# Nithin-Holla/meme_challenge

Measured on AMD Instinct MI355X. Metric: train samples/sec UNITER-base (36 regions, 128 tok), higher is better.
Workload: dtype f32

## Files before the change

### include/uniter_hip.h

```cpp
#ifndef UNITER_HIP_H
#define UNITER_HIP_H

#include <stddef.h>
#include <stdint.h>

#ifdef __cplusplus
extern "C" {
#endif

#define UNITER_ABI_VERSION 1

#define UNITER_E_ARG   (-1)
#define UNITER_E_SHAPE (-2)
#define UNITER_E_WS    (-3)
#define UNITER_E_STATE (-4)

int         uniter_abi_version(void);
const char* uniter_last_error(void);
const char* uniter_build_info(void);

enum {
  UNITER_EPI_NONE      = 0,
  UNITER_EPI_BIAS      = 1,
  UNITER_EPI_BIAS_GELU = 2,
// ... 67 lines not shown
                  void* stream);
int uniter_join3(const void* x3, int rows, int cols, size_t row_stride, size_t piece_stride, float* x, int ld,
                 void* stream);
int uniter_gemm_x3_cfg(int cfg, int nsplit, int a_kmajor, int b_kmajor, int M, int N, int K, const void* A, int lda,
                       int psa, const void* B, int ldb, int psb, float* C, int ldc, long c_split_stride, void* C_x3,
                       int ldcx, int pscx, int epilogue, const float* bias, const float* aux_in, float* aux_out,
                       int ld_aux, void* stream);
int uniter_gemm_x3_plan(int M, int N, int K, int avail_cus, int nsplit_fixed, int* cfg, int* nsplit);
int uniter_gemm_x3_plan_fwd32(int M, int N, int K, int avail_cus, int nsplit_fixed, int* cfg, int* nsplit);
int uniter_wgrad_x3_group(int cfg, int n, const int* M, const int* N, int K, const void* const* A,
                          const void* const* B, float* const* dW, int overwrite, int max_wgs, void* stream);
typedef struct uniter_x3_riders {
  double* ssq;
  float* colsum_out;
  int grid, njobs, nred;
  const float* part[4];
  int nparts[4], stride[4], n[4], seg[4];
  float* out[4][3];
  int first_item[5];
} uniter_x3_riders_t;
int uniter_gemm_x3_colpart(int cfg, int a_kmajor, int b_kmajor, int M, int N, int K, const void* A, int lda, int psa,
                           const void* B, int ldb, int psb, float* C, int ldc, void* C_x3, int ldcx, int pscx,
                           const float* aux_in, int ld_aux, float* colsum_part, void* stream);
int uniter_wgrad_x3_group_riders(int cfg, int n, const int* M, const int* N, int K, const void* const* A,
                                 const void* const* B, float* const* dW, int overwrite, int max_wgs,
                                 uniter_x3_riders_t* riders, void* stream);
int uniter_wgrad_x3_group_slots(int cfg, int n, const int* M, const int* N, int max_wgs);
size_t uniter_gemm_x3_balanced_ws_bytes(void);
int uniter_gemm_x3_cfg_ws(int cfg, int nsplit, int a_kmajor, int b_kmajor, int M, int N, int K, const void* A, int lda,
                          int psa, const void* B, int ldb, int psb, float* C, int ldc, long c_split_stride, void* C_x3,
                          int ldcx, int pscx, int epilogue, const float* bias, const float* aux_in, float* aux_out,
                          int ld_aux, void* ws, size_t ws_bytes, void* stream);
int uniter_wgrad_x3_group_ws(int cfg, int n, const int* M, const int* N, int K, const void* const* A,
                             const void* const* B, float* const* dW, int overwrite, int max_wgs,
                             uniter_x3_riders_t* riders, void* ws, size_t ws_bytes, void* stream);
int uniter_wgrad_x3_group_slots_ws(int cfg, int n, const int* M, const int* N, int K, int max_wgs, size_t ws_bytes);
int uniter_wgrad_bf16_group_riders(int cfg, int n, const int* M, const int* N, int K, const void* const* A,
                                   const void* const* B, float* const* dW, int overwrite, int max_wgs,
                                   uniter_x3_riders_t* riders, void* stream);
int uniter_wgrad_bf16_group_slots(int n, const int* M, const int* N, int max_wgs);
int uniter_wgrad_bf16_group_slots_cfg(int cfg, int n, const int* M, const int* N, int max_wgs);
int uniter_gemm_bf16p_plan(int M, int N, int K, int avail_cus, int nsplit_fixed, int b_kmajor, int* cfg, int* nsplit);
int uniter_gemm_bf16p_colpart(int b_kmajor, int M, int N, int K, const void* A, int lda, const void* B, int ldb, float* C, int ldc,
                              void* C_bf16, int ldcb, const void* aux_in, int aux_in_bf16, int ld_aux, float* colsum_part,
                              void* stream);
int uniter_colsum_x3_add(const void* x3, int rows, int cols, int ldx, float* out, void* stream);
// ... 426 lines not shown
```

### meme_challenge_amd/_lib.py

```python
import ctypes as C
import os

import torch

_HERE = os.path.dirname(os.path.abspath(__file__))
LIB_PATH = os.path.join(_HERE, 'libuniter_hip.so')
if os.environ.get('UNITER_LIB_VARIANT'):
    LIB_PATH = os.path.join(_HERE, 'libuniter_hip_%s.so' % os.environ['UNITER_LIB_VARIANT'])

c_f32p = C.c_void_p
c_i64p = C.c_void_p
c_u8p = C.c_void_p


class UniterConfigC(C.Structure):
    _fields_ = [('hidden_size', C.c_int32), ('num_hidden_layers', C.c_int32),
                ('num_attention_heads', C.c_int32), ('intermediate_size', C.c_int32),
                ('vocab_size', C.c_int32), ('max_position_embeddings', C.c_int32),
                ('type_vocab_size', C.c_int32), ('img_dim', C.c_int32),
                ('hidden_dropout_prob', C.c_float),
                ('attention_probs_dropout_prob', C.c_float)]


class X3RidersC(C.Structure):
# ... 50 lines not shown
    'uniter_slab_reduce_add': (_I, [_P, _I, _SZ, _P, _SZ, _P]),
    'uniter_colsum_bf16_add': (_I, [_P, _I, _I, _I, _P, _P]),
    'uniter_colsum_bf16_add_det': (_I, [_P, _I, _I, _I, _P, _P, _SZ, _P]),
    'uniter_colsum_det_ws_bytes': (_SZ, [_I, _I]),
    'uniter_wgrad_bf16_group': (_I, [_I, _I, _P, _P, _I, _P, _P, _P, _P]),
    'uniter_wgrad_f32_group': (_I, [_I, _P, _P, _I, _P, _P, _P, _I, _P]),
    'uniter_ln_bwd_b16': (_I, [_P, _P, _P, _P, _P, _P, _P, _P, _P, _P, _P, _I, _I, _F, _U64, _U32, _U32, _P, _SZ, _P]),
    'uniter_ln_bwd_rows': (_I, [_P, _P, _P, _P, _P, _P, _P, _P, _I, _I, _I, _F, _U64, _U32, _U32, _P, _SZ, _P]),
    'uniter_ln_bwd_finalize': (_I, [_P, _SZ, _I, _I, _P, _P, _P, _P]),
    'uniter_ln_bwd': (_I, [_P, _P, _P, _P, _P, _P, _P, _P, _P, _P, _I, _I, _F, _U64, _U32, _U32, _P, _SZ, _P]),
    'uniter_ln_bwd_ws_bytes': (_SZ, [_I, _I]),
    'uniter_attn_fwd': (_I, [_P, _P, _P, _P, _I, _I, _I, _F, _U64, _U32, _U32, _P]),
    'uniter_gemm_bf16res_cfg': (_I, [_I, _I, _I, _I, _I, _I, _P, _I, _P, _I, _P, _I, _P, _I, _I, _P, _P, _P, _I, _I, _P]),
    'uniter_gemm_bf16v2_cfg': (_I, [_I, _I, _I, _I, _I, _I, _I, _P, _I, _P, _I, _P, _I, C.c_long, _P, _I, _I, _P, _P, _I, _P, _I, _I, _I, _P]),
    'uniter_split3': (_I, [_P, _I, _I, _I, _P, _SZ, _SZ, _P]),
    'uniter_join3': (_I, [_P, _I, _I, _SZ, _SZ, _P, _I, _P]),
    'uniter_gemm_x3_cfg': (_I, [_I, _I, _I, _I, _I, _I, _I, _P, _I, _I, _P, _I, _I, _P, _I, C.c_long, _P, _I, _I, _I, _P, _P, _P, _I, _P]),
    'uniter_ln_fwd_slabs_x3': (_I, [_P, _I, _SZ, _P, _P, _P, _P, _P, _P, _P, _P, _I, _I, _F, _U64, _U32, _U32, _P]),
    'uniter_ln_bwd_rows_slabs_x3': (_I, [_P, _I, _SZ, _P, _P, _P, _P, _P, _P, _P, _I, _I, _I, _F, _U64, _U32, _U32, _P, _SZ, _P]),
    'uniter_wgrad_x3_group': (_I, [_I, _I, _P, _P, _I, _P, _P, _P, _I, _I, _P]),
    'uniter_gemm_x3_plan': (_I, [_I, _I, _I, _I, _I, _P, _P]),
    'uniter_gemm_x3_plan_fwd32': (_I, [_I, _I, _I, _I, _I, _P, _P]),
    'uniter_gemm_x3_colpart': (_I, [_I, _I, _I, _I, _I, _I, _P, _I, _I, _P, _I, _I, _P, _I, _P, _I, _I, _P, _I, _P, _P]),
    'uniter_wgrad_x3_group_riders': (_I, [_I, _I, _P, _P, _I, _P, _P, _P, _I, _I, _P, _P]),
    'uniter_wgrad_x3_group_slots': (_I, [_I, _I, _P, _P, _I]),
    'uniter_gemm_x3_balanced_ws_bytes': (_SZ, []),
    'uniter_gemm_x3_cfg_ws': (_I, [_I, _I, _I, _I, _I, _I, _I, _P, _I, _I, _P, _I, _I, _P, _I, C.c_long, _P, _I, _I, _I, _P, _P, _P, _I, _P, _SZ, _P]),
    'uniter_wgrad_x3_group_ws': (_I, [_I, _I, _P, _P, _I, _P, _P, _P, _I, _I, _P, _P, _SZ, _P]),
    'uniter_wgrad_x3_group_slots_ws': (_I, [_I, _I, _P, _P, _I, _I, _SZ]),
    'uniter_wgrad_bf16_group_riders': (_I, [_I, _I, _P, _P, _I, _P, _P, _P, _I, _I, _P, _P]),
    'uniter_wgrad_bf16_group_slots': (_I, [_I, _P, _P, _I]),
    'uniter_wgrad_bf16_group_slots_cfg': (_I, [_I, _I, _P, _P, _I]),
    'uniter_gemm_bf16p_plan': (_I, [_I, _I, _I, _I, _I, _I, _P, _P]),
    'uniter_gemm_bf16p_colpart': (_I, [_I, _I, _I, _I, _P, _I, _P, _I, _P, _I, _P, _I, _P, _I, _I, _P, _P]),
    'uniter_hidden_keep_bits_bytes': (_SZ, [_SZ]),
    'uniter_hidden_keep_bits_gen': (_I, [_P, _SZ, _I, _U32, _U32, _U32, _SZ, _F, _U64, _U32, _P]),
    'uniter_ln_set_next_keep_bits': (_I, [_P]),
    'uniter_model_set_norm_partials': (_I, [_P, _P, _SZ]),
    'uniter_model_set_aux_stream': (_I, [_P, _P]),
    'uniter_model_set_cu_reserve': (_I, [_P, _I]),
    'uniter_model_set_deterministic': (_I, [_P, _I]),
    'uniter_model_deterministic_coverage': (_I, [_P]),
    'uniter_attn_bwd_set_next_det': (_I, [_I]),
    'uniter_model_norm_partials_per_layer': (_I, [_P]),
    'uniter_colsum_x3_add': (_I, [_P, _I, _I, _I, _P, _P]),
    'uniter_colsum_x3_add_det': (_I, [_P, _I, _I, _I, _P, _P, _SZ, _P]),
# ... 223 lines not shown
```

### meme_challenge_amd/csrc/gemm_internal.h

```cpp
#pragma once
#include "common.h"

struct GemmOperand {
  const void* p = nullptr;
  int ld = 0, piece_stride = 0, kmajor = 0;
};
struct GemmCall {
  int M = 0, N = 0, K = 0;
  GemmOperand A, B;
  float* C = nullptr;
  int ldc = 0, nsplit = 1;
  long c_split_stride = 0;
  void* Ccopy = nullptr;
  int ld_copy = 0, ps_copy = 0;
  int epi = UNITER_EPI_NONE;
  const float* bias = nullptr;
  const void* aux_in = nullptr;
  void* aux_out = nullptr;
  int aux_in_bf16 = 0, aux_out_bf16 = 0, ld_aux = 0;
  int beta = 0, no_sk = 0;
  float* colpart = nullptr;
  void* sk_ws = nullptr;
  size_t sk_ws_bytes = 0;
  void* stream = nullptr;
// ... 12 lines not shown
  return 0;
}
static inline bool gemm_side_buffers_aligned(const GemmCall& c) {
  return c.ldc % 4 == 0 && c.ld_copy % 8 == 0 && c.ld_aux % 4 == 0 && ((uintptr_t)c.C & 15) == 0 && ((uintptr_t)c.Ccopy & 15) == 0 &&
         ((uintptr_t)c.aux_in & 15) == 0 && ((uintptr_t)c.aux_out & 15) == 0 && ((uintptr_t)c.bias & 15) == 0;
}
static inline bool gemm_f32_side_in_range(const GemmCall& c, int pad) {
  return ((size_t)c.M + pad) * (c.ldc > 0 ? c.ldc : 1) * 4 < (1ull << 31) && ((size_t)c.M + pad) * (c.ld_aux > 0 ? c.ld_aux : 1) * 4 < (1ull << 31);
}

int gemm_f32_run(int cfg, int tag, const GemmCall& c, const LaunchOpts& lo);
int gemm_bf16_run(int cfg, const GemmCall& c, const LaunchOpts& lo);
int gemm_bf16res_run(int cfg, const GemmCall& c, const LaunchOpts& lo);
int gemm_bf16v2_run(int cfg, const GemmCall& c, const LaunchOpts& lo);
int gemm_b1p_run(int cfg, const GemmCall& c, const LaunchOpts& lo);
int gemm_x3_run(int cfg, const GemmCall& c, const LaunchOpts& lo);
size_t gemm_x3_sk_ws_bytes();
int gemm_x3_wgrad_default_cfg();
int gemm_x3_pick_split(int M, int N, int K);
int gemm_x3_pick_split_on(int M, int N, int K, int avail, int cu_reserve);
int gemm_bf16v2_pick_split(int M, int N, int K);
int gemm_b1p_pick_split(int M, int N, int K, int avail, int cu_reserve);
int gemm_bf16v2_wgrad_pieces(int M, int N, int K);

struct WgradGroupCall {
  int n = 0, K = 0;
  const int* Kp = nullptr;
  const int *Mo = nullptr, *No = nullptr;
  const void *const *A = nullptr, *const *B = nullptr;
  float* const* dW = nullptr;
  int overwrite = 0, max_wgs = 0;
  uniter_x3_riders_t* riders = nullptr;
  void *sk_ws = nullptr, *stream = nullptr;
  size_t sk_ws_bytes = 0;
};
int gemm_f32_wgrad_group(const WgradGroupCall& c, const LaunchOpts& lo);
int gemm_bf16v2_wgrad_group(int cfg, const WgradGroupCall& c, const LaunchOpts& lo);
int gemm_b1p_wgrad_group(const WgradGroupCall& c, const LaunchOpts& lo);
int gemm_x3_wgrad_group(int cfg, const WgradGroupCall& c, const LaunchOpts& lo);
int gemm_x3_wgrad_group_slots(int cfg, int n, const int* Mo, const int* No, int max_wgs, int K, size_t sk_ws_bytes, int cu_reserve);
int gemm_x3_wgrad_group_balanced_wgs(int cfg, int n, const int* Mo, const int* No, int cu_reserve);
int gemm_b1p_wgrad_group_slots(int n, const int* Mo, const int* No, int max_wgs, int cu_reserve);
int gemm_bf16v2_wgrad_group_slots(int n, const int* Mo, const int* No, int max_wgs, int cu_reserve);
int gemm_bf16v2_wgrad_group_balanced_wgs(int n, const int* Mo, const int* No, int cu_reserve);

static inline int wgrad_group_check(const char* who, const WgradGroupCall& c) {
// ... 68 lines not shown
```

### meme_challenge_amd/csrc/model.cpp

```cpp
#include <stdlib.h>
#include <string.h>
#include <algorithm>
#include <string>
#include <vector>
#include "common.h"
#include "gemm_internal.h"
#include "philox.h"
#include "switches.h"

namespace {

enum { P_WORD = 0, P_POS, P_TYPE, P_ELN_G, P_ELN_B, P_IMG_W, P_IMG_B, P_ILN_G, P_ILN_B, P_PLN_G, P_PLN_B,
       P_POSL_W, P_POSL_B, P_MASK_EMB, P_FLN_G, P_FLN_B, P_LAYER0 };
enum { L_QW = 0, L_QB, L_KW, L_KB, L_VW, L_VB, L_OW, L_OB, L_LN1_G, L_LN1_B, L_W1, L_B1, L_W2, L_B2, L_LN2_G,
       L_LN2_B, L_COUNT };

const char* kEmbNames[P_LAYER0] = {
    "embeddings.word_embeddings.weight", "embeddings.position_embeddings.weight",
    "embeddings.token_type_embeddings.weight", "embeddings.LayerNorm.weight", "embeddings.LayerNorm.bias",
    "img_embeddings.img_linear.weight", "img_embeddings.img_linear.bias",
    "img_embeddings.img_layer_norm.weight", "img_embeddings.img_layer_norm.bias",
    "img_embeddings.pos_layer_norm.weight", "img_embeddings.pos_layer_norm.bias",
    "img_embeddings.pos_linear.weight", "img_embeddings.pos_linear.bias",
    "img_embeddings.mask_embedding.weight", "img_embeddings.LayerNorm.weight", "img_embeddings.LayerNorm.bias"};
// ... 37 lines not shown
  AttnKernel attn_fwd, attn_bwd;
  float *feat_eff, *imgfc, *img_stats, *cat, *emb;
  std::vector<LayerBufs> layers;
  float *dcat, *d_imgfc, *d_posfc, *d_feat, *dsum, *dpk;
  unsigned short* embb;
  Precision prec = PREC_F32;
  bool copies() const { return prec >= PREC_BF16; }
  int ns_kh;
  int ns_ki_b, ns_kh_b, ns_k3h_b;
  int ns_ki, ns_k3h;
  bool packed;
  bool det;
  int wg_group;
  float* wg_slabs;
  unsigned char* hid_keepb;
  size_t hid_stride;
  bool hid_on;
  void *ln_ws, *col_ws, *emb_ws, *attn_ws;
  void *emb_ws2, *emb_ws3;
  size_t ln_ws_bytes, col_ws_bytes, emb_ws_bytes, attn_ws_bytes;
  void *sk_main, *sk_side;
  size_t sk_bytes;
  bool head_rows = false;
  int hr_ns_h = 1, hr_ns_i = 1;
  LayerBufs hr;
  float *hr_x = nullptr, *hr_dy = nullptr;
  size_t total;
};

}

struct uniter_model {
  uniter_config_t cfg;
  int n_params;
  std::vector<float*> p, g;
  std::vector<std::string> names;
  std::vector<hipEvent_t> ev_main, ev_side, ev_mid;
  Precision precision = PREC_F32;
  bool mirror_paired = false;
  const unsigned short* mirror = nullptr;
  const float* mirror_base = nullptr;
  size_t mirror_numel = 0;
  const unsigned short* WB(int l, int k) const { return mirror + (LP(l, k) - mirror_base); }
  std::vector<hipEvent_t> ready;
  int prof_kind = 0;
  std::vector<hipEvent_t> prof_ev;
// ... 114 lines not shown
      b.dz2 = cv.f(M * H); b.g2 = cv.f(M * H); b.du = cv.f(M * I); b.dy1 = cv.f(s_ki_b * M * H); b.dz1 = cv.f(M * H);
      b.g1 = cv.f(M * H); b.dctx = cv.f(s_kh_b * M * H); b.dqkv = cv.f(M * 3 * H); b.delta = cv.f((size_t)B * nh * L);
      b.dx = cv.f(s_k3h * M * H);
      b.du_csum = cv.f((size_t)((M + 31) / 32) * I);
      b.qb_part = cv.f((size_t)B * 3 * H);
      b.keepb = (unsigned short*)cv.raw(uniter_attn_keep_bits_bytes(B, L, nh));
      b.ln_ws1 = cv.raw(uniter_ln_bwd_ws_bytes(pl.M, H));
      b.ln_ws2 = cv.raw(uniter_ln_bwd_ws_bytes(pl.M, H));
      if (pl.copies()) { b.g2b = cv.h(pc * M * H); b.dub = cv.h(pc * M * I); b.g1b = cv.h(pc * M * H); b.dqkvb = cv.h(pc * M * 3 * H); }
    }
  } else {
    LayerBufs base = LayerBufs();
    alloc_fwd(base);
    float* yB = cv.f(M * H);
    for (int l = 0; l < nl; ++l) {
      pl.layers[l] = base;
      if (l & 1) pl.layers[l].y2 = yB;
    }
  }
  pl.sk_bytes = gemm_x3_sk_ws_bytes();
  pl.sk_main = (x3 && (sw.x3_balanced & 2)) ? cv.raw(pl.sk_bytes) : nullptr;
  pl.sk_side = (x3 && save && (sw.x3_balanced & 1)) ? cv.raw(pl.sk_bytes) : nullptr;
  pl.head_rows = false;
  pl.hr = LayerBufs(); pl.hr_x = pl.hr_dy = nullptr;
  if (x3 && !pl.packed) {
    const size_t Bc = (size_t)B;
    LayerBufs& h = pl.hr;
    auto pieces_for = [](int K) { const int n = K / 32 / 2; return n < 1 ? 1 : (n > 8 ? 8 : n); };
    pl.hr_ns_h = pieces_for(H); pl.hr_ns_i = pieces_for(I);
    const size_t s_h = (size_t)pl.hr_ns_h, s_i = (size_t)pl.hr_ns_i;
    h.ctx = cv.f(Bc * H); h.ctxb = cv.h(pc * Bc * H); pl.hr_x = cv.f(Bc * H); h.t1 = cv.f(s_h * Bc * H);
    h.z1 = save ? cv.f(Bc * H) : nullptr; h.mean1 = cv.f(Bc); h.rstd1 = cv.f(Bc); h.y1 = cv.f(Bc * H); h.y1b = cv.h(pc * Bc * H);
    h.u = save ? cv.f(Bc * I) : nullptr; h.hact = cv.f(Bc * I); h.hactb = cv.h(pc * Bc * I); h.t2 = cv.f(s_i * Bc * H);
    h.z2 = save ? cv.f(Bc * H) : nullptr; h.mean2 = cv.f(Bc); h.rstd2 = cv.f(Bc); h.y2 = cv.f(Bc * H);
    if (save) {
      pl.hr_dy = cv.f(Bc * H); h.dz2 = cv.f(Bc * H); h.g2b = cv.h(pc * Bc * H); h.dub = cv.h(pc * Bc * I); h.dy1 = cv.f(s_i * Bc * H);
      h.dz1 = cv.f(Bc * H); h.g1b = cv.h(pc * Bc * H); h.dctx = cv.f(Bc * H);
      h.du_csum = cv.f((size_t)((Bc + 31) / 32) * I);
      h.ln_ws1 = cv.raw(uniter_ln_bwd_ws_bytes(B, H));
      h.ln_ws2 = cv.raw(uniter_ln_bwd_ws_bytes(B, H));
    }
  }
  if (save) {
    pl.hid_stride = align_up(uniter_hidden_keep_bits_bytes(M * H), 256);
    pl.hid_keepb = (unsigned char*)cv.raw(pl.hid_stride * 2 * nl);
    pl.dcat = cv.f((size_t)B * pl.S * H);
    pl.d_imgfc = cv.f(BR * H);
    pl.d_posfc = cv.f(BR * H);
    pl.d_feat = has_masks ? cv.f(BR * c.img_dim) : nullptr;
    pl.dsum = cv.f(M * H);
    pl.dpk = cv.f(M * H);
    pl.ln_ws_bytes = uniter_ln_bwd_ws_bytes(pl.M, H);
    pl.ln_ws = cv.raw(pl.ln_ws_bytes);
    const int maxN = 3 * H > I ? 3 * H : I;
    pl.col_ws_bytes = uniter_colsum_ws_bytes(pl.M, maxN);
    pl.col_ws = cv.raw(pl.col_ws_bytes);
    const int rows = B * (T > R ? T : R);
    pl.emb_ws_bytes = uniter_embed_bwd_ws_bytes(rows, H);
    pl.det = m->deterministic;
    if (pl.det) {
      const size_t d = uniter_embed_bwd_det_ws_bytes(has_txt ? B * T : 0, (int)BR, H);
      if (d > pl.emb_ws_bytes) pl.emb_ws_bytes = d;
    }
// ... 78 lines not shown
    const int cfg = (kind == UNITER_K_GEMM_FFN_UP_FWD && sw.x3_cfg_ffn_up_fwd) ? sw.x3_cfg_ffn_up_fwd : sw.x3_cfg;
    const LaunchOpts lo = {ps.stamp, sw.main_prio_x3, m->launch_reserve};
    g.A = {a.b, 3 * K, K, 0}; g.B.piece_stride = (int)m->mirror_numel; g.ld_copy = 3 * N; g.ps_copy = N; g.ld_aux = N;
    g.sk_ws = pl.sk_main; g.sk_ws_bytes = pl.sk_main ? pl.sk_bytes : 0;
    return gemm_x3_run(cfg | (m->mirror_paired ? 64 : 0), g, lo);
  }
  const LaunchOpts lo = {ps.stamp, sw.main_prio_bf16, m->launch_reserve};
  g.A = {a.b, K, 0, 0}; g.ld_copy = c.b ? N : 0; g.ld_aux = ld_aux;
  g.aux_in_bf16 = epi == UNITER_EPI_MUL || epi == UNITER_EPI_DGELU; g.aux_out_bf16 = epi == UNITER_EPI_BIAS_GELU || epi == UNITER_EPI_BIAS_GELU_D;
  int cfg = 0;
  const int mask = sw.b16_persist;
  const bool epi_ok = epi == UNITER_EPI_NONE || epi == UNITER_EPI_BIAS || epi == UNITER_EPI_ADD || epi == UNITER_EPI_BIAS_GELU_D || epi == UNITER_EPI_MUL;
  if (epi_ok && K % 64 == 0) {
    if ((mask & 1) && kind == UNITER_K_GEMM_QKV_FWD && !bkm && N % 192 == 0) cfg = 8;
    else if ((mask & 2) && pieces > 1 && N <= 1024) cfg = 6;
    else if ((mask & 8) && pieces == 1 && N >= 2048) cfg = 7;
  }
  if (colpart) {
    UCHECK_ARG(epi_ok && K % 64 == 0 && pieces == 1, "linear: column partials ride on the persistent kernels");
    return gemm_b1p_run(7, g, lo);
  }
  return gemm_bf16v2_run(cfg, g, lo);
}
AttnKernel attn_kernel(const Plan& pl, float p_drop, bool save, bool keep_pre, bool bwd) {
  const Switches& sw = uniter_switches();
  const bool fused = pl.L <= uniter_attn_varlen_max_len();
  const bool pieces = pl.L <= uniter_attn_x3_max_len() && (p_drop == 0.f || keep_pre || bwd);
  if (pl.prec == PREC_BF16 && fused) return (sw.attn_b16x && pieces) ? ATTN_B16X : ATTN_BF16_PRE;
  if (pl.prec == PREC_X3 && sw.attn_x3 && pieces && (fused || !bwd)) return ATTN_X3;
  if (pl.prec == PREC_X3 && fused) return ATTN_F32_PRE_X3;
  if (pl.packed || (save && fused)) return ATTN_F32_PRE;
  return ATTN_F32;
}
int x3_backward_cus(const uniter_model* m) {
  const int a = (gemm_chip_cus() - m->cu_reserve) / 8 * 8;
  return a >= 8 ? a : 8;
}
struct WgradGroup {
  bool riders = false;
  bool colpart = false;
  int cfg = 0, max_wgs = 0, slots = 0;
};
WgradGroup wgrad_group(const uniter_model* m, const Plan& pl, int l, int cu_reserve, bool own_k = false) {
  const Switches& sw = uniter_switches();
  const int H = m->cfg.hidden_size, I = m->cfg.intermediate_size;
  const int Mo[4] = {I, H, 3 * H, H}, No[4] = {H, I, H, H};
// ... 141 lines not shown
  if (pl.det) {
    const LayerBufs& lb = rows != pl.M ? pl.hr : pl.layers[l];
    return (x3 ? uniter_colsum_x3_add_det : uniter_colsum_bf16_add_det)(t.A[0], rows, t.Mo[0], t.Mo[0], m->LG(l, L_B1), lb.du_csum,
                                                                       du_csum_bytes(rows, t.Mo[0]), sd);
  }
  return (x3 ? uniter_colsum_x3_add : uniter_colsum_bf16_add)(t.A[0], rows, t.Mo[0], t.Mo[0], m->LG(l, L_B1), sd);
}

int head_rows_gather(void* dst, const void* src, int B, int L, size_t row_bytes, hipStream_t st) {
  UCHECK_HIP(hipMemcpy2DAsync(dst, row_bytes, src, (size_t)L * row_bytes, row_bytes, (size_t)B, hipMemcpyDeviceToDevice, st));
  return 0;
}
int head_rows_scatter(void* dst, const void* src, int B, int L, size_t row_bytes, hipStream_t st) {
  UCHECK_HIP(hipMemcpy2DAsync(dst, (size_t)L * row_bytes, src, row_bytes, row_bytes, (size_t)B, hipMemcpyDeviceToDevice, st));
  return 0;
}
int head_rows_forward(uniter_model* m, hipStream_t st, int l, Act x, float* hidden_out, float ph) {
  Plan& pl = m->plan;
  const int H = m->cfg.hidden_size, I = m->cfg.intermediate_size, B = pl.B, L = pl.L;
  const LayerBufs& lb = pl.layers[l];
  LayerBufs& h = pl.hr;
  const bool save = pl.mode != 0;
  const size_t rowb = (size_t)H * sizeof(float);
  UCHECK_RC(head_rows_gather(h.ctx, lb.ctx, B, L, rowb, st));
  UCHECK_RC(head_rows_gather(pl.hr_x, x.f, B, L, rowb, st));
  const Act ctx = {h.ctx, h.ctxb}, y1 = {h.y1, h.y1b}, hact = {h.hact, h.hactb};
  UCHECK_RC(operand_copy(pl, ctx, B, H, st));
  UCHECK_RC(linear(m, UNITER_K_GEMM_ATTN_OUT_FWD, st, 0, B, H, H, l, L_OW, ctx, Act{h.t1, nullptr}, pl.hr_ns_h, UNITER_EPI_BIAS, m->LP(l, L_OB), nullptr,
                   nullptr));
  UCHECK_RC(ln_fwd(m, st, l, 0, h.t1, pl.hr_ns_h, pl.hr_x, h.z1, y1, h.mean1, h.rstd1, ph, B, L));
  float* gelu_aux = save ? h.u : h.hact;
  UCHECK_RC(linear(m, UNITER_K_GEMM_FFN_UP_FWD, st, 0, B, I, H, l, L_W1, y1, hact, 1, UNITER_EPI_BIAS_GELU_D, m->LP(l, L_B1), nullptr, gelu_aux));
  UCHECK_RC(linear(m, UNITER_K_GEMM_FFN_DOWN_FWD, st, 0, B, H, I, l, L_W2, hact, Act{h.t2, nullptr}, pl.hr_ns_i, UNITER_EPI_BIAS, m->LP(l, L_B2), nullptr,
                   nullptr));
  UCHECK_RC(ln_fwd(m, st, l, 1, h.t2, pl.hr_ns_i, h.y1, h.z2, Act{h.y2, nullptr}, h.mean2, h.rstd2, ph, B, L));
  UCHECK_HIP(hipMemsetAsync(hidden_out, 0, (size_t)B * L * rowb, st));
  return head_rows_scatter(hidden_out, h.y2, B, L, rowb, st);
}

int validate_batch(const uniter_model* m, const uniter_batch_t* b) {
  UCHECK_ARG(b, "batch is NULL");
  UCHECK_ARG(b->B > 0 && b->L > 0, "batch: B and L must be positive");
  UCHECK_ARG(b->input_ids || b->img_feat, "batch: need input_ids and/or img_feat");
  UCHECK_ARG(b->attention_mask, "batch: attention_mask is NULL");
  if (b->input_ids) UCHECK_ARG(b->position_ids && b->T > 0, "batch: text needs position_ids and T > 0");
  if (b->img_feat) UCHECK_ARG(b->img_pos_feat && b->R > 0, "batch: image needs img_pos_feat and R > 0");
  const int S = (b->input_ids ? b->T : 0) + (b->img_feat ? b->R : 0);
  if (!(b->input_ids && b->img_feat && b->gather_index))
    UCHECK_SHAPE(b->L == S || (b->input_ids && b->img_feat && b->L <= S),
                 "batch: without gather_index L (%d) must equal T+R (%d)", b->L, S);
  UCHECK_SHAPE(b->T <= m->cfg.max_position_embeddings || !b->input_ids, "batch: T exceeds max_position_embeddings");
  return 0;
}

}

extern "C" int uniter_num_params(const uniter_config_t* cfg) {
// ... 347 lines not shown
  const float* dh = nullptr;
  if (l == nl - 1 || m->all_layers) {
    dh = m->d_hidden + (m->all_layers ? (size_t)l * ((size_t)B * L * H) : 0);
    if (pl.packed) {
      UCHECK_RC(uniter_row_gather(dh, m->batch.pack_dst, pl.dpk, M, H, B * L, st));
      dh = pl.dpk;
    }
  }
  const bool hr = pl.head_rows && l == nl - 1;
  LayerBufs& pb = hr ? pl.hr : lb;
  const int Mp = hr ? B : M, row_step = hr ? L : 1;
  if (hr) {
    UCHECK_RC(head_rows_gather(pl.hr_dy, dh, B, L, (size_t)H * sizeof(float), st));
    dy = pl.hr_dy;
  } else if (l == nl - 1) {
    dy = dh;
  } else if (m->all_layers) {
    UCHECK_RC(launch_add_f32(pl.dsum, pl.layers[l + 1].dx, dh, MH, st));
    dy = pl.dsum;
  } else {
    dy = pl.layers[l + 1].dx;
  }
  const bool copies = pl.copies();
  const Act g2 = {ph > 0.f ? (copies ? nullptr : pb.g2) : pb.dz2, pb.g2b};
  const Act g1 = {ph > 0.f ? (copies ? nullptr : pb.g1) : pb.dz1, pb.g1b};
  const int ns_dy = (l == nl - 1 || m->all_layers) ? 1 : pl.ns_k3h;
  const int ns_dx = (l == 0 || m->all_layers) ? 1 : pl.ns_k3h;
  UCHECK_RC(ln_bwd(m, st, l, 1, dy, ns_dy, pb.z2, pb.mean2, pb.rstd2, pb.dz2, g2, pb.ln_ws2, ph, hr ? Mp : 0, row_step));
  const bool fuse_db1 = H % 64 == 0;
  const Switches& sw = uniter_switches();
  const bool attn_b16 = attn_is_b16(pl.attn_bwd);
  const bool fused_qb = pl.attn_bwd != ATTN_F32;
  const int ns_dctx = hr ? 1 : (pl.attn_bwd == ATTN_X3 && sw.dctx_split) ? pl.ns_kh_b : 1;
  const int ns_dy1 = hr ? pl.hr_ns_i : pl.ns_ki_b;
  const int epi_du = pl.gelu_d ? UNITER_EPI_MUL : UNITER_EPI_DGELU;
  const WgradGroup wg = copies ? wgrad_group(m, pl, l, m->launch_reserve, hr && Mp != M) : WgradGroup();
  const Act du = {pb.du, pb.dub}, dqkv = {lb.dqkv, lb.dqkvb};
  UCHECK_RC(linear(m, UNITER_K_GEMM_DGRAD, st, 1, Mp, I, H, l, L_W2, g2, du, 1, epi_du, nullptr, pb.u, nullptr,
                   (copies ? wg.colpart : fuse_db1) ? pb.du_csum : nullptr));
  UCHECK_RC(linear(m, UNITER_K_GEMM_DGRAD, st, 1, Mp, H, I, l, L_W1, du, Act{pb.dy1, nullptr}, ns_dy1, UNITER_EPI_ADD, nullptr, pb.dz2,
                   nullptr));
  UCHECK_RC(ln_bwd(m, st, l, 0, pb.dy1, ns_dy1, pb.z1, pb.mean1, pb.rstd1, pb.dz1, g1, pb.ln_ws1, ph, hr ? Mp : 0, row_step));
  const WgradProducts wp = {{I, H, 3 * H, H}, {H, I, H, H}, {pb.dub, pb.g2b, lb.dqkvb, pb.g1b}, {pb.y1b, pb.hactb, x.b, pb.ctxb},
                            {m->LG(l, L_W1), m->LG(l, L_W2), m->LG(l, L_QW), m->LG(l, L_OW)}, {Mp, Mp, M, Mp}};
  const int wp_all[4] = {0, 1, 2, 3}, wp_early[3] = {0, 1, 3}, wp_late[1] = {2};
  const bool wg_early = pl.prec == PREC_BF16 && pl.wg_group >= 2 && sd != st;
  if (wg_early) {
    UCHECK_HIP(hipEventRecord(m->ev_mid[l], st));
    UCHECK_HIP(hipStreamWaitEvent(sd, m->ev_mid[l], 0));
    UCHECK_RC(wgrad_launch(m, l, sd, wp, wp_early, 3, 1, 0, nullptr, true));
  }
  UCHECK_RC(linear(m, UNITER_K_GEMM_DGRAD, st, 1, Mp, H, H, l, L_OW, g1, Act{pb.dctx, nullptr}, ns_dctx, UNITER_EPI_NONE, nullptr, nullptr,
                   nullptr));
  if (hr) {
    const size_t rowb = (size_t)H * sizeof(float);
    UCHECK_HIP(hipMemsetAsync(lb.dctx, 0, MH * sizeof(float), st));
    UCHECK_RC(head_rows_scatter(lb.dctx, pb.dctx, B, L, rowb, st));
    UCHECK_HIP(hipMemsetAsync(lb.dz1, 0, MH * sizeof(float), st));
    UCHECK_RC(head_rows_scatter(lb.dz1, pb.dz1, B, L, rowb, st));
  }
  if (m->ag.out) {
    const uniter_model::AttnGrads& ag = m->ag;
    UCHECK_RC(uniter_attn_grad(lb.qkv, attn_b16 ? 1 : 0, pl.packed ? nullptr : m->batch.attention_mask, pl.packed ? m->batch.cu_seqlens : nullptr,
                               lb.dctx, ns_dctx, MH, ag.out + (size_t)l * ag.stride,
                               ag.head_sums ? ag.head_sums + (size_t)l * B * nh : nullptr, ag.ws, ag.ws_bytes, B, L, nh, ag.reduce, st));
  }
  {
    ProfScope ps(m, UNITER_K_ATTN_BWD, st);
    const AttnKernel k = pl.attn_bwd;
    const bool flags_only = attn_reads_flags_only(k);
    AttnCall c;
    c.B = B; c.L = L; c.nh = nh; c.qkv = lb.qkv; c.qkv_is_bf16 = attn_b16;
    c.mask = pl.packed ? nullptr : m->batch.attention_mask; c.cu_seqlens = pl.packed ? m->batch.cu_seqlens : nullptr;
    c.ctx = lb.ctx; c.lse = lb.lse; c.p_drop = pa; c.stream = st;
    c.keep_bits = fused_qb ? lb.keepb : nullptr;
    c.seed = flags_only ? 0 : m->seed; c.offset = flags_only ? 0 : m->offset; c.site = flags_only ? 0 : SITE_ATTN_PROBS(l);
// ... 462 lines not shown
```

Before: 1701.

## Add skinny fp32 MFMA GEMM for head-rows last-layer linears

Adds a dedicated skinny GEMM kernel (M<=64) that uses fp32 MFMA with per-wave k-splitting and an LDS reduction, with fused bias/GELU/add/mul epilogues. The last layer's head-rows path uses it for forward and dgrad linears on the few gathered rows. It reads ctx straight through a strided lda, which removes a gather and an operand split copy. The intent is to cut launch and tiling overhead of general GEMMs on tiny-M shapes. In exchange it allocates extra fp32 gradient buffers and adds a second code path whose accuracy and x3 copy handling must match the old one.

```diff
diff --git a/include/uniter_hip.h b/include/uniter_hip.h
--- a/include/uniter_hip.h
+++ b/include/uniter_hip.h
@@ -113,6 +113,9 @@
 int uniter_gemm_x3_colpart(int cfg, int a_kmajor, int b_kmajor, int M, int N, int K, const void* A, int lda, int psa,
                            const void* B, int ldb, int psb, float* C, int ldc, void* C_x3, int ldcx, int pscx,
                            const float* aux_in, int ld_aux, float* colsum_part, void* stream);
+int uniter_gemm_skinny(int b_kmajor, int M, int N, int K, const float* A, int lda, const float* W, int ldw, float* C, int ldc,
+                       long c_split_stride, int nsplit, void* C_x3, int ldcx, int pscx, int epilogue, const float* bias,
+                       const float* aux_in, float* aux_out, int ld_aux, float* colsum_part, void* stream);
 int uniter_wgrad_x3_group_riders(int cfg, int n, const int* M, const int* N, int K, const void* const* A,
                                  const void* const* B, float* const* dW, int overwrite, int max_wgs,
                                  uniter_x3_riders_t* riders, void* stream);
diff --git a/meme_challenge_amd/_lib.py b/meme_challenge_amd/_lib.py
--- a/meme_challenge_amd/_lib.py
+++ b/meme_challenge_amd/_lib.py
@@ -96,6 +96,7 @@
     'uniter_gemm_x3_plan': (_I, [_I, _I, _I, _I, _I, _P, _P]),
     'uniter_gemm_x3_plan_fwd32': (_I, [_I, _I, _I, _I, _I, _P, _P]),
     'uniter_gemm_x3_colpart': (_I, [_I, _I, _I, _I, _I, _I, _P, _I, _I, _P, _I, _I, _P, _I, _P, _I, _I, _P, _I, _P, _P]),
+    'uniter_gemm_skinny': (_I, [_I, _I, _I, _I, _P, _I, _P, _I, _P, _I, C.c_long, _I, _P, _I, _I, _I, _P, _P, _P, _I, _P, _P]),
     'uniter_wgrad_x3_group_riders': (_I, [_I, _I, _P, _P, _I, _P, _P, _P, _I, _I, _P, _P]),
     'uniter_wgrad_x3_group_slots': (_I, [_I, _I, _P, _P, _I]),
     'uniter_gemm_x3_balanced_ws_bytes': (_SZ, []),
diff --git a/meme_challenge_amd/csrc/gemm_internal.h b/meme_challenge_amd/csrc/gemm_internal.h
--- a/meme_challenge_amd/csrc/gemm_internal.h
+++ b/meme_challenge_amd/csrc/gemm_internal.h
@@ -58,6 +58,9 @@
 int gemm_bf16v2_pick_split(int M, int N, int K);
 int gemm_b1p_pick_split(int M, int N, int K, int avail, int cu_reserve);
 int gemm_bf16v2_wgrad_pieces(int M, int N, int K);
+int gemm_skinny_run(const GemmCall& c, const LaunchOpts& lo);
+bool gemm_skinny_takes(int M, int N, int K);
+int gemm_skinny_pick_split(int K);
 
 struct WgradGroupCall {
   int n = 0, K = 0;
diff --git a/meme_challenge_amd/csrc/head_rows.hip b/meme_challenge_amd/csrc/head_rows.hip
--- /dev/null
+++ b/meme_challenge_amd/csrc/head_rows.hip
@@ -0,0 +1,208 @@
+#include "bf16_tile.h"
+#include "gemm_internal.h"
+
+namespace {
+
+constexpr int SK_WAVES = 8;
+
+struct SkArgs {
+  int M, N, K;
+  const float* A; int lda;
+  const float* W; int ldw;
+  float* C; int ldc; long c_split_stride; int nsplit;
+  unsigned short* Cx; int ldcx, pscx;
+  const float* bias; const float* aux_in; float* aux_out; int ld_aux;
+  float* colpart;
+  int strips;
+  unsigned long long* stamp;
+};
+
+enum { SK_NONE = 0, SK_BIAS, SK_BIAS_GELU_D, SK_ADD, SK_MUL };
+
+__device__ __forceinline__ f32x4 ld4(const float* p, bool ok) {
+  return ok ? *reinterpret_cast<const f32x4*>(p) : f32x4{0.f, 0.f, 0.f, 0.f};
+}
+
+template <int BKM, int RB>
+__global__ __launch_bounds__(64 * SK_WAVES) void skinny_kernel(const SkArgs g, const int epi) {
+  constexpr int SN = BKM ? 32 : 16, KU = BKM ? 16 : 32, NB = BKM ? 2 : 1, ROWS = 16 * RB;
+  __shared__ __attribute__((aligned(16))) float part[SK_WAVES * ROWS * SN];
+  const int lane = threadIdx.x & 63, wave = threadIdx.x >> 6, r = lane & 15, q = lane >> 4;
+  const int piece = blockIdx.x / g.strips, n0 = (blockIdx.x - piece * g.strips) * SN;
+  stamp_begin(g.stamp);
+  const int units = (g.K + KU - 1) / KU;
+  const int u0 = (int)((long)units * piece / g.nsplit), u1 = (int)((long)units * (piece + 1) / g.nsplit);
+  f32x4 acc[RB][NB];
+#pragma unroll
+  for (int b = 0; b < RB; ++b)
+#pragma unroll
+    for (int j = 0; j < NB; ++j) acc[b][j] = f32x4{0.f, 0.f, 0.f, 0.f};
+#if defined(__HIP_DEVICE_COMPILE__)
+  if constexpr (!BKM) {
+    const int n = n0 + r;
+    const float* wrow = g.W + (size_t)(n < g.N ? n : 0) * g.ldw;
+#pragma unroll 2
+    for (int u = u0 + wave; u < u1; u += SK_WAVES) {
+      const int k = u * 32 + q * 8;
+      const bool ok0 = k < g.K, ok1 = k + 4 < g.K;
+      const f32x4 w0 = ld4(wrow + k, ok0 && n < g.N), w1 = ld4(wrow + k + 4, ok1 && n < g.N);
+      f32x4 a0[RB], a1[RB];
+#pragma unroll
+      for (int b = 0; b < RB; ++b) {
+        const int m = 16 * b + r;
+        const float* arow = g.A + (size_t)(m < g.M ? m : 0) * g.lda;
+        a0[b] = ld4(arow + k, ok0 && m < g.M); a1[b] = ld4(arow + k + 4, ok1 && m < g.M);
+      }
+#pragma unroll
+      for (int e = 0; e < 4; ++e)
+#pragma unroll
+        for (int b = 0; b < RB; ++b) acc[b][0] = __builtin_amdgcn_mfma_f32_16x16x4f32(a0[b][e], w0[e], acc[b][0], 0, 0, 0);
+#pragma unroll
+      for (int e = 0; e < 4; ++e)
+#pragma unroll
+        for (int b = 0; b < RB; ++b) acc[b][0] = __builtin_amdgcn_mfma_f32_16x16x4f32(a1[b][e], w1[e], acc[b][0], 0, 0, 0);
+    }
+  } else {
+    typedef float f32x2 __attribute__((ext_vector_type(2)));
+    const int n = n0 + 2 * r;
+#pragma unroll 2
+    for (int u = u0 + wave; u < u1; u += SK_WAVES) {
+      const int k = u * 16 + q * 4;
+      const bool ok = k < g.K;
+      f32x2 w[4];
+#pragma unroll
+      for (int t = 0; t < 4; ++t)
+        w[t] = (ok && n < g.N) ? *reinterpret_cast<const f32x2*>(g.W + (size_t)(k + t) * g.ldw + n) : f32x2{0.f, 0.f};
+      f32x4 a[RB];
+#pragma unroll
+      for (int b = 0; b < RB; ++b) {
+        const int m = 16 * b + r;
+        a[b] = ld4(g.A + (size_t)(m < g.M ? m : 0) * g.lda + k, ok && m < g.M);
+      }
+#pragma unroll
+      for (int t = 0; t < 4; ++t)
+#pragma unroll
+        for (int b = 0; b < RB; ++b)
+#pragma unroll
+          for (int j = 0; j < 2; ++j) acc[b][j] = __builtin_amdgcn_mfma_f32_16x16x4f32(a[b][t], w[t][j], acc[b][j], 0, 0, 0);
+    }
+  }
+#endif
+#pragma unroll
+  for (int b = 0; b < RB; ++b)
+#pragma unroll
+    for (int j = 0; j < NB; ++j)
+#pragma unroll
+      for (int e = 0; e < 4; ++e) part[(wave * ROWS + 16 * b + 4 * q + e) * SN + NB * r + j] = acc[b][j][e];
+  __syncthreads();
+  const bool first = piece == 0;
+  float* const Cs = g.C ? g.C + (size_t)piece * g.c_split_stride : nullptr;
+  for (int it = threadIdx.x; it < g.M * (SN / 2); it += 64 * SK_WAVES) {
+    const int m = it / (SN / 2), c = 2 * (it - m * (SN / 2)), n = n0 + c;
+    float v0 = part[m * SN + c], v1 = part[m * SN + c + 1];
+#pragma unroll
+    for (int w = 1; w < SK_WAVES; ++w) { v0 += part[(w * ROWS + m) * SN + c]; v1 += part[(w * ROWS + m) * SN + c + 1]; }
+    if (n < g.N && first) {
+      if (epi == SK_BIAS || epi == SK_BIAS_GELU_D) { v0 += g.bias[n]; v1 += g.bias[n + 1]; }
+      if (epi == SK_BIAS_GELU_D) {
+        float y0, d0, y1, d1;
+        gelu_pair_fast(v0, y0, d0); gelu_pair_fast(v1, y1, d1);
+        if (g.aux_out) { g.aux_out[(size_t)m * g.ld_aux + n] = d0; g.aux_out[(size_t)m * g.ld_aux + n + 1] = d1; }
+        v0 = y0; v1 = y1;
+      } else if (epi == SK_ADD) {
+        v0 += g.aux_in[(size_t)m * g.ld_aux + n]; v1 += g.aux_in[(size_t)m * g.ld_aux + n + 1];
+      } else if (epi == SK_MUL) {
+        v0 *= g.aux_in[(size_t)m * g.ld_aux + n]; v1 *= g.aux_in[(size_t)m * g.ld_aux + n + 1];
+      }
+    }
+    if (n < g.N) {
+      if (Cs) { Cs[(size_t)m * g.ldc + n] = v0; Cs[(size_t)m * g.ldc + n + 1] = v1; }
+      if (g.Cx) {
+        unsigned w1, w2, w3;
+        split3_pair(v0, v1, w1, w2, w3);
+        unsigned short* o = g.Cx + (size_t)m * g.ldcx + n;
+        *reinterpret_cast<unsigned*>(o) = w1;
+        *reinterpret_cast<unsigned*>(o + g.pscx) = w2;
+        *reinterpret_cast<unsigned*>(o + 2 * (size_t)g.pscx) = w3;
+      }
+    }
+    if (g.colpart) { part[m * SN + c] = v0; part[m * SN + c + 1] = v1; }
+  }
+  if (g.colpart) {
+    __syncthreads();
+    const int c = threadIdx.x, n = n0 + c;
+    if (c < SN && n < g.N) {
+      float s = 0.f;
+      for (int m = 0; m < g.M; ++m) s += part[m * SN + c];
+      g.colpart[n] = s;
+    }
+  }
+  stamp_end(g.stamp);
+}
+
+template <int BKM>
+int skinny_launch(const SkArgs& g, int epi, hipStream_t st) {
+  const int rb = (g.M + 15) / 16;
+  const dim3 grid(g.strips * g.nsplit), block(64 * SK_WAVES);
+  switch (rb) {
+    case 1: skinny_kernel<BKM, 1><<<grid, block, 0, st>>>(g, epi); break;
+    case 2: skinny_kernel<BKM, 2><<<grid, block, 0, st>>>(g, epi); break;
+    case 3: skinny_kernel<BKM, 3><<<grid, block, 0, st>>>(g, epi); break;
+    default: skinny_kernel<BKM, 4><<<grid, block, 0, st>>>(g, epi); break;
+  }
+  UCHECK_LAUNCH();
+  return 0;
+}
+
+}
+
+int gemm_skinny_pick_split(int K) {
+  const int n = K / 256;
+  return n < 1 ? 1 : (n > 8 ? 8 : n);
+}
+
+bool gemm_skinny_takes(int M, int N, int K) { return M >= 1 && M <= 64 && N >= 8 && N % 8 == 0 && K >= 4 && K % 4 == 0; }
+
+int gemm_skinny_run(const GemmCall& c, const LaunchOpts& lo) {
+  const int M = c.M, N = c.N, K = c.K, epilogue = c.epi;
+  UCHECK_ARG(M > 0 && N > 0 && K > 0 && c.A.p && c.B.p && (c.C || c.Ccopy), "gemm_skinny: bad argument");
+  UCHECK_ARG(!c.A.kmajor && !c.A.piece_stride && !c.B.piece_stride && !c.beta && !c.aux_in_bf16 && !c.aux_out_bf16 && !c.sk_ws,
+             "gemm_skinny: fp32 operands, activations k-contiguous, no accumulate, fp32 aux operands, no workspace");
+  UCHECK_ARG(c.nsplit >= 1 && c.nsplit <= 8 && (c.nsplit == 1 || (c.C && !c.Ccopy && !c.colpart && c.c_split_stride >= (long)M * c.ldc)),
+             "gemm_skinny: k-pieces need fp32 slabs (no x3 output, no column sums)");
+  int epi = -1;
+  switch (epilogue) {
+    case UNITER_EPI_NONE: epi = SK_NONE; break;
+    case UNITER_EPI_BIAS: epi = SK_BIAS; break;
+    case UNITER_EPI_BIAS_GELU_D: epi = SK_BIAS_GELU_D; break;
+    case UNITER_EPI_ADD: epi = SK_ADD; break;
+    case UNITER_EPI_MUL: epi = SK_MUL; break;
+    default: break;
+  }
+  UCHECK_ARG(epi >= 0, "gemm_skinny: epilogue %d not built (none, bias, bias + gelu with gelu' out, + aux, x aux)", epilogue);
+  UCHECK_ARG(c.nsplit == 1 || epi == SK_NONE || epi == SK_BIAS || epi == SK_ADD,
+             "gemm_skinny: k-pieces only under an epilogue that adds (slab 0 carries it): none, bias, + aux");
+  UCHECK_RC(gemm_check_epilogue("gemm_skinny", c, GEMM_EPI_PERSISTENT, false));
+  UCHECK_SHAPE(gemm_skinny_takes(M, N, K), "gemm_skinny: M <= 64, N %% 8 == 0 and K %% 4 == 0 required (M=%d N=%d K=%d)", M, N, K);
+  const bool aux = epi == SK_ADD || epi == SK_MUL || (epi == SK_BIAS_GELU_D && c.aux_out);
+  UCHECK_SHAPE(c.A.ld >= K && c.A.ld % 4 == 0 && c.B.ld >= (c.B.kmajor ? N : K) && c.B.ld % 4 == 0 && (!c.C || (c.ldc >= N && c.ldc % 2 == 0)) &&
+               (!c.Ccopy || (c.ld_copy >= N && c.ld_copy % 8 == 0 && c.ps_copy >= 0 && c.ps_copy % 8 == 0)) && (!aux || c.ld_aux >= N) &&
+               ((uintptr_t)c.A.p & 15) == 0 && ((uintptr_t)c.B.p & 15) == 0 && ((uintptr_t)c.C & 7) == 0 && ((uintptr_t)c.Ccopy & 3) == 0 &&
+               ((uintptr_t)c.bias & 3) == 0 && ((uintptr_t)c.aux_in & 3) == 0 && ((uintptr_t)c.aux_out & 3) == 0 && ((uintptr_t)c.colpart & 3) == 0,
+               "gemm_skinny: leading dimensions (operands %% 4, x3 strides %% 8) and 16-byte aligned operands required");
+  const SkArgs g = {M, N, K, (const float*)c.A.p, c.A.ld, (const float*)c.B.p, c.B.ld, c.C, c.ldc, c.c_split_stride, c.nsplit,
+                    (unsigned short*)c.Ccopy, c.ld_copy, c.ps_copy, c.bias, (const float*)c.aux_in, (float*)c.aux_out, c.ld_aux, c.colpart,
+                    (N + (c.B.kmajor ? 32 : 16) - 1) / (c.B.kmajor ? 32 : 16), lo.stamp};
+  hipStream_t st = (hipStream_t)c.stream;
+  return c.B.kmajor ? skinny_launch<1>(g, epi, st) : skinny_launch<0>(g, epi, st);
+}
+
+extern "C" int uniter_gemm_skinny(int b_kmajor, int M, int N, int K, const float* A, int lda, const float* W, int ldw, float* C, int ldc,
+                                  long c_split_stride, int nsplit, void* C_x3, int ldcx, int pscx, int epilogue, const float* bias,
+                                  const float* aux_in, float* aux_out, int ld_aux, float* colsum_part, void* stream) {
+  GemmCall c;
+  c.M = M; c.N = N; c.K = K; c.A = {A, lda, 0, 0}; c.B = {W, ldw, 0, b_kmajor != 0};
+  c.C = C; c.ldc = ldc; c.c_split_stride = c_split_stride; c.nsplit = nsplit; c.Ccopy = C_x3; c.ld_copy = ldcx; c.ps_copy = pscx;
+  c.epi = epilogue; c.bias = bias; c.aux_in = aux_in; c.aux_out = aux_out; c.ld_aux = ld_aux; c.colpart = colsum_part; c.stream = stream;
+  return gemm_skinny_run(c, LaunchOpts{});
+}
diff --git a/meme_challenge_amd/csrc/model.cpp b/meme_challenge_amd/csrc/model.cpp
--- a/meme_challenge_amd/csrc/model.cpp
+++ b/meme_challenge_amd/csrc/model.cpp
@@ -83,6 +83,7 @@
   void *sk_main, *sk_side;
   size_t sk_bytes;
   bool head_rows = false;
+  bool hr_skinny = false;
   int hr_ns_h = 1, hr_ns_i = 1;
   LayerBufs hr;
   float *hr_x = nullptr, *hr_dy = nullptr;
@@ -243,12 +244,14 @@
   pl.sk_main = (x3 && (sw.x3_balanced & 2)) ? cv.raw(pl.sk_bytes) : nullptr;
   pl.sk_side = (x3 && save && (sw.x3_balanced & 1)) ? cv.raw(pl.sk_bytes) : nullptr;
   pl.head_rows = false;
-  pl.hr = LayerBufs(); pl.hr_x = pl.hr_dy = nullptr;
+  pl.hr = LayerBufs(); pl.hr_x = pl.hr_dy = nullptr; pl.hr_skinny = false;
   if (x3 && !pl.packed) {
     const size_t Bc = (size_t)B;
     LayerBufs& h = pl.hr;
     auto pieces_for = [](int K) { const int n = K / 32 / 2; return n < 1 ? 1 : (n > 8 ? 8 : n); };
-    pl.hr_ns_h = pieces_for(H); pl.hr_ns_i = pieces_for(I);
+    pl.hr_skinny = (H >= 512 || I >= 512) && gemm_skinny_takes(B, H, I) && gemm_skinny_takes(B, I, H);
+    pl.hr_ns_h = pl.hr_skinny ? gemm_skinny_pick_split(H) : pieces_for(H);
+    pl.hr_ns_i = pl.hr_skinny ? gemm_skinny_pick_split(I) : pieces_for(I);
     const size_t s_h = (size_t)pl.hr_ns_h, s_i = (size_t)pl.hr_ns_i;
     h.ctx = cv.f(Bc * H); h.ctxb = cv.h(pc * Bc * H); pl.hr_x = cv.f(Bc * H); h.t1 = cv.f(s_h * Bc * H);
     h.z1 = save ? cv.f(Bc * H) : nullptr; h.mean1 = cv.f(Bc); h.rstd1 = cv.f(Bc); h.y1 = cv.f(Bc * H); h.y1b = cv.h(pc * Bc * H);
@@ -260,6 +263,7 @@
       h.du_csum = cv.f((size_t)((Bc + 31) / 32) * I);
       h.ln_ws1 = cv.raw(uniter_ln_bwd_ws_bytes(B, H));
       h.ln_ws2 = cv.raw(uniter_ln_bwd_ws_bytes(B, H));
+      if (pl.hr_skinny) { h.g2 = cv.f(Bc * H); h.du = cv.f(Bc * I); h.g1 = cv.f(Bc * H); }
     }
   }
   if (save) {
@@ -384,6 +388,15 @@
   }
   return gemm_bf16v2_run(cfg, g, lo);
 }
+int skinny(uniter_model* m, int kind, hipStream_t st, int bkm, int M, int N, int K, int l, int w, const float* a, Act c, int pieces, int epi,
+           const float* bias, const float* aux_in, float* aux_out, float* colpart = nullptr, int lda = 0) {
+  ProfScope ps(m, kind, st);
+  GemmCall g;
+  g.M = M; g.N = N; g.K = K; g.A = {a, lda > 0 ? lda : K, 0, 0}; g.B = {m->LP(l, w), bkm ? N : K, 0, bkm}; g.C = c.f; g.ldc = N; g.c_split_stride = (long)M * N;
+  g.nsplit = pieces; g.Ccopy = c.b; g.ld_copy = 3 * N; g.ps_copy = N; g.epi = epi; g.bias = bias; g.aux_in = aux_in; g.aux_out = aux_out;
+  g.ld_aux = N; g.colpart = colpart; g.stream = st;
+  return gemm_skinny_run(g, LaunchOpts{ps.stamp, 0, m->launch_reserve});
+}
 AttnKernel attn_kernel(const Plan& pl, float p_drop, bool save, bool keep_pre, bool bwd) {
   const Switches& sw = uniter_switches();
   const bool fused = pl.L <= uniter_attn_varlen_max_len();
@@ -571,17 +584,28 @@
   LayerBufs& h = pl.hr;
   const bool save = pl.mode != 0;
   const size_t rowb = (size_t)H * sizeof(float);
-  UCHECK_RC(head_rows_gather(h.ctx, lb.ctx, B, L, rowb, st));
   UCHECK_RC(head_rows_gather(pl.hr_x, x.f, B, L, rowb, st));
   const Act ctx = {h.ctx, h.ctxb}, y1 = {h.y1, h.y1b}, hact = {h.hact, h.hactb};
-  UCHECK_RC(operand_copy(pl, ctx, B, H, st));
-  UCHECK_RC(linear(m, UNITER_K_GEMM_ATTN_OUT_FWD, st, 0, B, H, H, l, L_OW, ctx, Act{h.t1, nullptr}, pl.hr_ns_h, UNITER_EPI_BIAS, m->LP(l, L_OB), nullptr,
-                   nullptr));
-  UCHECK_RC(ln_fwd(m, st, l, 0, h.t1, pl.hr_ns_h, pl.hr_x, h.z1, y1, h.mean1, h.rstd1, ph, B, L));
-  float* gelu_aux = save ? h.u : h.hact;
-  UCHECK_RC(linear(m, UNITER_K_GEMM_FFN_UP_FWD, st, 0, B, I, H, l, L_W1, y1, hact, 1, UNITER_EPI_BIAS_GELU_D, m->LP(l, L_B1), nullptr, gelu_aux));
-  UCHECK_RC(linear(m, UNITER_K_GEMM_FFN_DOWN_FWD, st, 0, B, H, I, l, L_W2, hact, Act{h.t2, nullptr}, pl.hr_ns_i, UNITER_EPI_BIAS, m->LP(l, L_B2), nullptr,
-                   nullptr));
+  if (pl.hr_skinny) {
+    if (save) UCHECK_RC(uniter_split3(lb.ctx, B, H, L * H, h.ctxb, (size_t)3 * H, (size_t)H, st));
+    UCHECK_RC(skinny(m, UNITER_K_GEMM_ATTN_OUT_FWD, st, 0, B, H, H, l, L_OW, lb.ctx, Act{h.t1, nullptr}, pl.hr_ns_h, UNITER_EPI_BIAS, m->LP(l, L_OB),
+                     nullptr, nullptr, nullptr, L * H));
+    UCHECK_RC(ln_fwd(m, st, l, 0, h.t1, pl.hr_ns_h, pl.hr_x, h.z1, y1, h.mean1, h.rstd1, ph, B, L));
+    UCHECK_RC(skinny(m, UNITER_K_GEMM_FFN_UP_FWD, st, 0, B, I, H, l, L_W1, h.y1, hact, 1, UNITER_EPI_BIAS_GELU_D, m->LP(l, L_B1), nullptr,
+                     save ? h.u : nullptr));
+    UCHECK_RC(skinny(m, UNITER_K_GEMM_FFN_DOWN_FWD, st, 0, B, H, I, l, L_W2, h.hact, Act{h.t2, nullptr}, pl.hr_ns_i, UNITER_EPI_BIAS, m->LP(l, L_B2),
+                     nullptr, nullptr));
+  } else {
+    UCHECK_RC(head_rows_gather(h.ctx, lb.ctx, B, L, rowb, st));
+    UCHECK_RC(operand_copy(pl, ctx, B, H, st));
+    UCHECK_RC(linear(m, UNITER_K_GEMM_ATTN_OUT_FWD, st, 0, B, H, H, l, L_OW, ctx, Act{h.t1, nullptr}, pl.hr_ns_h, UNITER_EPI_BIAS, m->LP(l, L_OB), nullptr,
+                     nullptr));
+    UCHECK_RC(ln_fwd(m, st, l, 0, h.t1, pl.hr_ns_h, pl.hr_x, h.z1, y1, h.mean1, h.rstd1, ph, B, L));
+    float* gelu_aux = save ? h.u : h.hact;
+    UCHECK_RC(linear(m, UNITER_K_GEMM_FFN_UP_FWD, st, 0, B, I, H, l, L_W1, y1, hact, 1, UNITER_EPI_BIAS_GELU_D, m->LP(l, L_B1), nullptr, gelu_aux));
+    UCHECK_RC(linear(m, UNITER_K_GEMM_FFN_DOWN_FWD, st, 0, B, H, I, l, L_W2, hact, Act{h.t2, nullptr}, pl.hr_ns_i, UNITER_EPI_BIAS, m->LP(l, L_B2), nullptr,
+                     nullptr));
+  }
   UCHECK_RC(ln_fwd(m, st, l, 1, h.t2, pl.hr_ns_i, h.y1, h.z2, Act{h.y2, nullptr}, h.mean2, h.rstd2, ph, B, L));
   UCHECK_HIP(hipMemsetAsync(hidden_out, 0, (size_t)B * L * rowb, st));
   return head_rows_scatter(hidden_out, h.y2, B, L, rowb, st);
@@ -975,8 +999,9 @@
     dy = pl.layers[l + 1].dx;
   }
   const bool copies = pl.copies();
-  const Act g2 = {ph > 0.f ? (copies ? nullptr : pb.g2) : pb.dz2, pb.g2b};
-  const Act g1 = {ph > 0.f ? (copies ? nullptr : pb.g1) : pb.dz1, pb.g1b};
+  const bool sk = hr && pl.hr_skinny;
+  const Act g2 = {ph > 0.f ? ((copies && !sk) ? nullptr : pb.g2) : pb.dz2, pb.g2b};
+  const Act g1 = {ph > 0.f ? ((copies && !sk) ? nullptr : pb.g1) : pb.dz1, pb.g1b};
   const int ns_dy = (l == nl - 1 || m->all_layers) ? 1 : pl.ns_k3h;
   const int ns_dx = (l == 0 || m->all_layers) ? 1 : pl.ns_k3h;
   UCHECK_RC(ln_bwd(m, st, l, 1, dy, ns_dy, pb.z2, pb.mean2, pb.rstd2, pb.dz2, g2, pb.ln_ws2, ph, hr ? Mp : 0, row_step));
@@ -989,10 +1014,15 @@
   const int epi_du = pl.gelu_d ? UNITER_EPI_MUL : UNITER_EPI_DGELU;
   const WgradGroup wg = copies ? wgrad_group(m, pl, l, m->launch_reserve, hr && Mp != M) : WgradGroup();
   const Act du = {pb.du, pb.dub}, dqkv = {lb.dqkv, lb.dqkvb};
-  UCHECK_RC(linear(m, UNITER_K_GEMM_DGRAD, st, 1, Mp, I, H, l, L_W2, g2, du, 1, epi_du, nullptr, pb.u, nullptr,
-                   (copies ? wg.colpart : fuse_db1) ? pb.du_csum : nullptr));
-  UCHECK_RC(linear(m, UNITER_K_GEMM_DGRAD, st, 1, Mp, H, I, l, L_W1, du, Act{pb.dy1, nullptr}, ns_dy1, UNITER_EPI_ADD, nullptr, pb.dz2,
-                   nullptr));
+  if (sk) {
+    UCHECK_RC(skinny(m, UNITER_K_GEMM_DGRAD, st, 1, Mp, I, H, l, L_W2, g2.f, du, 1, epi_du, nullptr, pb.u, nullptr, wg.colpart ? pb.du_csum : nullptr));
+    UCHECK_RC(skinny(m, UNITER_K_GEMM_DGRAD, st, 1, Mp, H, I, l, L_W1, pb.du, Act{pb.dy1, nullptr}, ns_dy1, UNITER_EPI_ADD, nullptr, pb.dz2, nullptr));
+  } else {
+    UCHECK_RC(linear(m, UNITER_K_GEMM_DGRAD, st, 1, Mp, I, H, l, L_W2, g2, du, 1, epi_du, nullptr, pb.u, nullptr,
+                     (copies ? wg.colpart : fuse_db1) ? pb.du_csum : nullptr));
+    UCHECK_RC(linear(m, UNITER_K_GEMM_DGRAD, st, 1, Mp, H, I, l, L_W1, du, Act{pb.dy1, nullptr}, ns_dy1, UNITER_EPI_ADD, nullptr, pb.dz2,
+                     nullptr));
+  }
   UCHECK_RC(ln_bwd(m, st, l, 0, pb.dy1, ns_dy1, pb.z1, pb.mean1, pb.rstd1, pb.dz1, g1, pb.ln_ws1, ph, hr ? Mp : 0, row_step));
   const WgradProducts wp = {{I, H, 3 * H, H}, {H, I, H, H}, {pb.dub, pb.g2b, lb.dqkvb, pb.g1b}, {pb.y1b, pb.hactb, x.b, pb.ctxb},
                             {m->LG(l, L_W1), m->LG(l, L_W2), m->LG(l, L_QW), m->LG(l, L_OW)}, {Mp, Mp, M, Mp}};
@@ -1003,8 +1033,9 @@
     UCHECK_HIP(hipStreamWaitEvent(sd, m->ev_mid[l], 0));
     UCHECK_RC(wgrad_launch(m, l, sd, wp, wp_early, 3, 1, 0, nullptr, true));
   }
-  UCHECK_RC(linear(m, UNITER_K_GEMM_DGRAD, st, 1, Mp, H, H, l, L_OW, g1, Act{pb.dctx, nullptr}, ns_dctx, UNITER_EPI_NONE, nullptr, nullptr,
-                   nullptr));
+  if (sk) UCHECK_RC(skinny(m, UNITER_K_GEMM_DGRAD, st, 1, Mp, H, H, l, L_OW, g1.f, Act{pb.dctx, nullptr}, ns_dctx, UNITER_EPI_NONE, nullptr, nullptr, nullptr));
+  else UCHECK_RC(linear(m, UNITER_K_GEMM_DGRAD, st, 1, Mp, H, H, l, L_OW, g1, Act{pb.dctx, nullptr}, ns_dctx, UNITER_EPI_NONE, nullptr, nullptr,
+                        nullptr));
   if (hr) {
     const size_t rowb = (size_t)H * sizeof(float);
     UCHECK_HIP(hipMemsetAsync(lb.dctx, 0, MH * sizeof(float), st));
```

After: 1723 (median of 6 runs). 1.01x the previous value.
